# tchen-research/new_cg_variants

Hardware: NVIDIA B200
Metric: CG iterations/s (pr_pcg, Jacobi, 3-D Poisson 256^3) (higher is better)
Workload: dtype f64

## Files before the change

### new_cg_variants_b200/csrc/cgx.cu

```cuda
#include <dlfcn.h>

#include "cgx_launch.cuh"

typedef CUresult (*EncodeTiledFn)(CUtensorMap*, CUtensorMapDataType, cuuint32_t, void*, const cuuint64_t*,
                                  const cuuint64_t*, const cuuint32_t*, const cuuint32_t*,
                                  CUtensorMapInterleave, CUtensorMapSwizzle, CUtensorMapL2promotion,
                                  CUtensorMapFloatOOBfill);
static EncodeTiledFn get_encode_tiled() {
  static EncodeTiledFn fn = nullptr;
  if (!fn) {
    void* p = nullptr;
    cudaDriverEntryPointQueryResult q;
    if (cudaGetDriverEntryPoint("cuTensorMapEncodeTiled", &p, cudaEnableDefault, &q) == cudaSuccess &&
        q == cudaDriverEntryPointSuccess)
      fn = (EncodeTiledFn)p;
  }
  return fn;
}

static thread_local std::string g_err;


int cgx_fail(int code, const char* fmt, ...) {
  char buf[512];
// ... 399 lines not shown

void launch_halo_push(cgx_ctx* c, Args g, const double* v, int ch) { launch_halo_push2(c, g, v, nullptr, ch); }
void launch_halo_push2(cgx_ctx* c, Args g, const double* v0, const double* v1, int ch) {
  if (c->dist.world <= 1) return;
  Plan p;
  p.hout_n = v1 ? 2 : 1; p.hout_ch = ch;
  plan_apply(c, g, p);
  g.halo_ll = 0;
  const double* vs[2] = {v0, v1};
  for (int i = 0; i < p.hout_n; ++i) {
    g.hout_ch = ch + i;
    g.hout_n = 1;
    if (c->dist.csr) {
      const int total = c->dist.send_ptr[c->dist.world];
      if (total > 0) { csr_halo_push_kernel<<<grid_for(c, total), kBlock, 0, c->stream>>>(g, vs[i]); c->launches++; }
    } else {
      halo_push_kernel<<<grid_for(c, c->dist.plane), kBlock, 0, c->stream>>>(g, vs[i]);
      c->launches++;
    }
  }
  plan_commit(c, g, p);
}

bool tma_encode_dims(double* ptr, i64 nx, i64 ny, i64 nz, CUtensorMap* out) {
  EncodeTiledFn enc = get_encode_tiled();
  if (!enc || !ptr) return false;
  cuuint64_t gdim[3] = {(cuuint64_t)nx, (cuuint64_t)ny, (cuuint64_t)nz};
  cuuint64_t gstr[2] = {(cuuint64_t)nx * 8, (cuuint64_t)nx * ny * 8};
  cuuint32_t box[3] = {(cuuint32_t)kPX, (cuuint32_t)kPY, 1};
  cuuint32_t estr[3] = {1, 1, 1};
  return enc(out, CU_TENSOR_MAP_DATA_TYPE_FLOAT64, 3, ptr, gdim, gstr, box, estr,
             CU_TENSOR_MAP_INTERLEAVE_NONE, CU_TENSOR_MAP_SWIZZLE_NONE,
             CU_TENSOR_MAP_L2_PROMOTION_L2_256B, CU_TENSOR_MAP_FLOAT_OOB_FILL_NONE) == CUDA_SUCCESS;
}

static bool tma_prepare_geom(cgx_ctx* c) {
  if (c->op_kind != 2 || c->no_tma) return false;
  const StencilOp& S = c->sten;
  if (S.nx % 2 != 0 || S.nx < 2) return false;
  if (S.ny < 4 && S.nz > 1) return false;
  if (!get_encode_tiled()) return false;
  TmaGeom& G = c->geom;
  G.nx = S.nx; G.ny = S.ny; G.nz = S.nz;
  G.ntx = (S.nx + kTX - 1) / kTX; G.nty = (S.ny + kTY - 1) / kTY;
  G.has_zlo = S.has_zlo; G.has_zhi = S.has_zhi;
  G.diag = S.diag; G.off = S.off;
  G.err = c->d_tma_err;
  G.nchunk = 1;
  G.march_y = 0;
  if (S.nz == 1 && !S.has_zlo && !S.has_zhi && G.nty > 1) {
    G.march_y = 1;
    G.nz = G.nty;
// ... 392 lines not shown
                c->tmap_ok[variant == CGX_CG ? V_R : V_W] &&
                c->pm != 1 && !c->no_elide && !(variant == CGX_GV && (gv_sched || c->gv_manual));
  c->launches_run = 0; c->loop_ms = 0.0;
  c->pend.clear();
  c->pr_fused = false; c->fpar = 0;
  for (int ch = 0; ch < 3; ++ch) c->hepoch[ch] = std::max(c->hepoch[ch], c->fepoch);
  if ((variant == CGX_PR || variant == CGX_M) && path == CGX_PATH_STREAM && !c->no_fused) {
    int frc = cgx_fused_prepare(c);
    if (frc) return frc;
  }
  return CGX_OK;
}

static int begin_finish(cgx_ctx* c, i64 launches0) {
  CU(cudaSetDevice(c->device));
  CU(cudaStreamSynchronize(c->stream));
  CU(cudaGetLastError());
  float ms0 = 0.f;
  CU(cudaEventElapsedTime(&ms0, c->ev[0], c->ev[1]));
  c->setup_ms = ms0;
  if (c->profile) { c->prof_cls.clear(); c->prof_used = 0; }
  c->launches_run = c->launches - launches0;
  c->ran = true;
  return CGX_OK;
}

static int check_device_flags(cgx_ctx* c, const char* who) {
  if (c->use_tma || c->op_kind == 1) {
    int flag = 0;
    CU(cudaMemcpy(&flag, c->d_tma_err, sizeof(int), cudaMemcpyDeviceToHost));
    if (flag) return fail(CGX_ERR_CUDA, "%s: an in-kernel pipeline wait (TMA plane copy / CSR product slot) did not complete within 1 s", who);
  }
  if (c->dist.world > 1 && c->d_win) {
    int err = 0;
    CU(cudaMemcpy(&err, c->d_win + offsetof(WinHdr, error), sizeof(int), cudaMemcpyDeviceToHost));
    if (err) return fail(CGX_ERR_CUDA, "%s: rank %d waited more than 10 s for a peer (halo or scalar exchange)",
                         who, c->dist.rank);
  }
  return CGX_OK;
}

static int group_begin(cgx_ctx** cs, int count, int variant, int max_iter, unsigned hist_mask, int path) {
  for (int i = 0; i < count; ++i)
    if (cs[i] && cs[i]->dist.world > 1 && cs[i]->tol > 0.0)
      return fail(CGX_ERR_UNSUPPORTED, "cgx_begin: a tolerance stops single-GPU solves only (rank %d of a partition has one set)",
                  cs[i]->dist.rank);
// ... 344 lines not shown
  Scal h;
  CU(cudaMemcpy(&h, c->d_sc + c->scpar, sizeof(Scal), cudaMemcpyDeviceToHost));
  info->setup_ms = c->setup_ms; info->loop_ms = c->loop_ms;
  info->h2d_bytes = 0; info->d2h_bytes = 0;
  info->kernel_launches = c->launches_run;
  info->iterations = c->cur_k;
  info->breakdown_iter = h.breakdown;
  info->path = c->path;
  info->stop_iter = c->stop_k;
  return CGX_OK;
}

extern "C" int cgx_set_option(cgx_ctx* c, const char* name, int value) {
  if (!c || !name) return fail(CGX_ERR_ARG, "cgx_set_option: bad arguments");
  if (!strcmp(name, "tma")) { c->no_tma = (value == 0); return CGX_OK; }
  if (!strcmp(name, "csr_stream")) { c->no_csr_stream = (value == 0); return CGX_OK; }
  if (!strcmp(name, "csr_bulk")) { c->csr_bulk = value; return CGX_OK; }
  if (!strcmp(name, "csr_bulk_ring")) { c->csr_bulk_ring = std::max(0, std::min(value, (int)kCbMaxRing)); return CGX_OK; }
  if (!strcmp(name, "csr_bulk_sum")) { c->csr_bulk_sum = value; return CGX_OK; }
  if (!strcmp(name, "csr_bulk_ctas")) { c->csr_bulk_ctas = std::max(1, std::min(value, 4)); return CGX_OK; }
  if (!strcmp(name, "csr_slab")) { c->no_slab = (value == 0); return CGX_OK; }
  if (!strcmp(name, "cg_elide")) { c->no_elide = (value == 0); return CGX_OK; }
  if (!strcmp(name, "pr_fused")) { c->no_fused = (value == 0); return CGX_OK; }
  if (!strcmp(name, "gv_manual")) { c->gv_manual = value != 0; return CGX_OK; }
  if (!strcmp(name, "fused_min_planes")) { c->fused_min_planes = std::max(1, value); return CGX_OK; }
  if (!strcmp(name, "pdl")) { c->pdl_mode = value; return CGX_OK; }
  if (!strcmp(name, "l2_keep")) { c->l2_keep = value; return CGX_OK; }
  if (!strcmp(name, "fused_min_slab")) { c->fused_min_slab = std::max(1, value); return CGX_OK; }
  if (!strcmp(name, "fused_chunks")) { c->fused_chunks = std::max(0, value); return CGX_OK; }
  if (!strcmp(name, "persistent_threshold")) { c->pers_threshold = value; return CGX_OK; }
  if (!strcmp(name, "pers_threads")) { c->pers_threads = value; return CGX_OK; }
  if (!strcmp(name, "pers_ctas")) { c->pers_ctas = value; return CGX_OK; }
  if (!strcmp(name, "debug_skip")) { c->dbg = value; return CGX_OK; }
  if (!strcmp(name, "tma_min_planes")) { c->tma_min_planes = value; return CGX_OK; }
  if (!strcmp(name, "ew_one_wave")) { c->one_wave = value != 0; return CGX_OK; }
  if (!strcmp(name, "stub_allreduce")) {
    if (c->dist.world <= 1) return fail(CGX_ERR_ARG, "cgx_set_option: stub_allreduce needs a partitioned run");
    if (value) { if (c->dist.mode != 3) { c->dist.saved_mode = c->dist.mode; c->dist.mode = 3; } }
    else if (c->dist.mode == 3) c->dist.mode = c->dist.saved_mode;
    return CGX_OK;
  }
  return fail(CGX_ERR_ARG, "cgx_set_option: unknown option '%s'", name);
}

extern "C" int cgx_set_tolerance(cgx_ctx* c, double rtol) {
  if (!c) return fail(CGX_ERR_ARG, "cgx_set_tolerance: ctx is NULL");
// ... 106 lines not shown
  if (info) *info = tmp;
  return tmp.breakdown_iter >= 0 ? CGX_ERR_BREAKDOWN : CGX_OK;
}

static int fetch(cgx_ctx* c, double* x, double* hist, cudaMemcpyKind kind) {
  if (!c || !c->ran) return fail(CGX_ERR_ARG, "cgx_fetch: nothing has been run");
  CU(cudaSetDevice(c->device));
  if (x) CU(cudaMemcpyAsync(x, c->vec[V_X], sizeof(double) * c->n, kind, c->stream));
  if (hist) CU(cudaMemcpyAsync(hist, c->d_hist, sizeof(double) * CGX_HIST_ROWS * (size_t)c->hist_len, kind, c->stream));
  CU(cudaStreamSynchronize(c->stream));
  return CGX_OK;
}
extern "C" int cgx_fetch_host(cgx_ctx* c, double* x, double* hist) { return fetch(c, x, hist, cudaMemcpyDeviceToHost); }
extern "C" int cgx_fetch_dev(cgx_ctx* c, double* x, double* hist) { return fetch(c, x, hist, cudaMemcpyDeviceToDevice); }

extern "C" int cgx_fetch_vector_host(cgx_ctx* c, const char* name, double* out) {
  if (!c || !c->ran || !name || !out) return fail(CGX_ERR_ARG, "cgx_fetch_vector_host: bad arguments");
  for (int i = 0; i < V_COUNT; ++i)
    if (!strcmp(name, kVecNames[i])) {
      if (!c->vec[i]) return fail(CGX_ERR_ARG, "cgx_fetch_vector_host: vector '%s' is not part of the last variant's state", name);
      CU(cudaSetDevice(c->device));
      if (((i == V_RT && c->variant == CGX_CG) || (i == V_WT && c->variant == CGX_GV)) && c->cg_elide && c->cur_k > 0) {
        launch_scale(c, c->d_dinv, c->vec[i == V_RT ? V_R : V_W], c->vec[i]);
        CU(cudaStreamSynchronize(c->stream));
      }
      CU(cudaMemcpy(out, cgx_cur_vec(c, i), sizeof(double) * c->n, cudaMemcpyDeviceToHost));
      return CGX_OK;
    }
  return fail(CGX_ERR_ARG, "cgx_fetch_vector_host: unknown vector '%s'", name);
}

extern "C" int cgx_solve_host(cgx_ctx* c, int variant, const double* b, const double* x0,
                              const double* xt, int64_t n, int max_iter, unsigned hist_mask,
                              int path, double* x, double* hist, cgx_info* info) {
  int rc = load_problem(c, b, x0, xt, n, cudaMemcpyHostToDevice);
  if (rc) return rc;
  int rrc = cgx_run(c, variant, max_iter, hist_mask, path, info);
  if (rrc != CGX_OK && rrc != CGX_ERR_BREAKDOWN) return rrc;
  rc = cgx_fetch_host(c, x, hist);
  if (rc) return rc;
  if (info) {
    info->h2d_bytes = (double)sizeof(double) * n * (xt ? 3 : 2);
    info->d2h_bytes = (double)sizeof(double) * ((x ? n : 0) + (hist ? (i64)CGX_HIST_ROWS * max_iter : 0));
  }
  return rrc;
}
// ... 169 lines not shown
```

### new_cg_variants_b200/csrc/cgx_fused.cu

```cuda
#include "cgx_host.h"
#include "cgx_stencil_fused.cuh"

static const int kFusedVec[3] = {V_P, V_S, V_RT};

double* cgx_cur_vec(cgx_ctx* c, int v) {
  if (c->pr_fused && (c->fpar & 1))
    for (int j = 0; j < 3; ++j)
      if (kFusedVec[j] == v) return c->alt[j];
  return c->vec[v];
}

int cgx_fused_prepare(cgx_ctx* c) {
  c->pr_fused = false;
  c->fpar = 0;
  if (c->op_kind != 2 || !c->use_tma || c->pm == 1) return CGX_OK;
  if (c->dist.world > 1 && (c->dist.mode == 2 || !c->halo_ll)) return CGX_OK;
  if (c->dist.world > 1 && c->sten.nz < c->fused_min_slab) return CGX_OK;
  const StencilOp& S = c->sten;
  for (int j = 0; j < 3; ++j) {
    if (!c->alt[j]) CU(cudaMalloc(&c->alt[j], sizeof(double) * c->n));
    if (!tma_encode_dims(c->vec[kFusedVec[j]], S.nx, S.ny, S.nz, &c->ftmap[0][j])) return CGX_OK;
    if (!tma_encode_dims(c->alt[j], S.nx, S.ny, S.nz, &c->ftmap[1][j])) return CGX_OK;
  }
  for (int ch = 0; ch < 3; ++ch) c->fepoch = std::max(c->fepoch, c->hepoch[ch]);
  if (c->dist.world > 1 && !c->d_gscr) CU(cudaMalloc(&c->d_gscr, sizeof(double) * 4 * (size_t)c->dist.plane));
  c->pr_fused = true;
  return CGX_OK;
}

template <int PM, bool MEUR, bool DIST>
static void launch_fused_t(cgx_ctx* c, const Args& g, int cur) {
  const size_t smem = fused_smem_bytes();
  const int per_sm = ctx_occupancy(c, (const void*)pr_fused_kernel<PM, MEUR, DIST>, kFThreads, smem);
  TmaGeom G = c->geom;
  const int cap = per_sm * c->sm_count, ncols = G.ntx * G.nty;
  G.nchunk = std::max(1, std::min(cap / std::max(1, ncols), G.nz / std::max(1, c->fused_min_planes)));
  if (c->fused_chunks > 0) G.nchunk = std::min(c->fused_chunks, G.nz);
  const int grid = (int)std::min<i64>((i64)ncols * G.nchunk, cap);
  launch_k(pr_fused_kernel<PM, MEUR, DIST>, grid, kFThreads, smem, c->stream, use_pdl(c), c->ftmap[cur][0], c->ftmap[cur][1],
           c->ftmap[cur][2], G, g);
}

void cgx_launch_pr_fused(cgx_ctx* c, Args g) {
  const int cur = c->fpar, nxt = cur ^ 1;
  g.p = nxt ? c->alt[0] : c->vec[V_P];
  g.s = nxt ? c->alt[1] : c->vec[V_S];
  g.rt = nxt ? c->alt[2] : c->vec[V_RT];
  const bool dist = c->dist.world > 1;
  g.gscr = c->d_gscr;
  Plan p;
  p.consume = true;
  p.produce = FK_PIPE;
  plan_apply(c, g, p);
  if (dist) {
    g.hin_epoch = c->fepoch; g.hin_par = (int)(g.hin_epoch & 1);
    g.hout_epoch = c->fepoch + 1; g.hout_par = (int)(g.hout_epoch & 1);
  }
  {
    ProfScope ps(c, PC_FUSED);
    const bool meur = c->variant == CGX_M;
#define CGX_FUSED_GO(PM, D) do { if (meur) launch_fused_t<PM, true, D>(c, g, cur); else launch_fused_t<PM, false, D>(c, g, cur); } while (0)
    if (c->pm == 2) { if (dist) CGX_FUSED_GO(2, true); else CGX_FUSED_GO(2, false); }
    else { if (dist) CGX_FUSED_GO(0, true); else CGX_FUSED_GO(0, false); }
// ... 18 lines not shown
```

### new_cg_variants_b200/csrc/cgx_host.h

```cpp
#pragma once
#include <cuda_runtime.h>

#include <algorithm>
#include <cmath>
#include <cstdarg>
#include <cstdio>
#include <cstring>
#include <functional>
#include <map>
#include <string>
#include <type_traits>
#include <utility>
#include <vector>

#include "../../include/cgx.h"
#include "cgx_kernels.cuh"
#include "cgx_stencil_tma.cuh"
#include "cgx_csr_bulk.cuh"
#include "cgx_persistent.cuh"

using namespace cgx;

int cgx_fail(int code, const char* fmt, ...);
#define fail cgx_fail
// ... 89 lines not shown
  bool peer_ipc[kMaxWorld] = {};
  bool dist_ready = false;
  cudaStream_t own_stream = nullptr;
  u64 epoch = 0;
  u64 hepoch[kChan] = {};
  u64 fepoch = 0;
  int scpar = 0;
  struct Pend { u64 e; int kind; int k; };
  std::vector<Pend> pend;
  void* nccl_comm = nullptr;
  cudaStream_t comm_stream = nullptr;
  cudaEvent_t ev_prod[kSlots] = {}, ev_red[kSlots] = {};
  double* d_nccl = nullptr;
  double* d_ppart = nullptr;
  u64* d_pbar = nullptr;
  PersOut* d_pout = nullptr;
  void* d_prank = nullptr;
  void* d_pbatch = nullptr;
  size_t pbatch_bytes = 0;
  double* d_exp[2][2] = {};
  int pers_threshold = 1 << 19;
  int pers_threads = 0, pers_ctas = 0;
  bool pr_fused = false, no_fused = false;
  int fpar = 0;
  double* alt[3] = {};
  double* d_gscr = nullptr;
  CUtensorMap ftmap[2][3];
  int pdl_mode = 1;
  int l2_keep = -1;
  int fused_min_slab = 64;
  int fused_min_planes = 8, fused_chunks = 0;
  unsigned capture = 0, capture_req = 0;
  double* d_cap[3] = {};
  std::vector<uint8_t> gv_replace;
  bool gv_manual = false;
  int cur_stage = 0;
  std::map<std::pair<const void*, size_t>, int> occ;
  int* d_tma_err = nullptr;
  int variant = 0, max_iter = 0, cur_k = 0, path = CGX_PATH_STREAM;
  double tol = 0.0, run_tol = 0.0;
  int stop_k = -1;
  int* h_stop = nullptr;
  cudaEvent_t ev_stop[2] = {nullptr, nullptr};
  i64 launches_run = 0;
  double setup_ms = 0.0, loop_ms = 0.0;
};
// ... 38 lines not shown
VecIn vec_in(cgx_ctx* c, const double* v, int ch, const Args& g);

int ctx_occupancy(cgx_ctx* c, const void* fn, int threads, size_t smem);

template <class... KArgs, class... Args>
inline cudaError_t launch_k(void (*kern)(KArgs...), int grid, int block, size_t smem, cudaStream_t st, bool pdl, Args&&... args) {
  cudaLaunchConfig_t cfg = {};
  cfg.gridDim = dim3(grid); cfg.blockDim = dim3(block); cfg.dynamicSmemBytes = smem; cfg.stream = st;
  cudaLaunchAttribute at[1];
  at[0].id = cudaLaunchAttributeProgrammaticStreamSerialization;
  at[0].val.programmaticStreamSerializationAllowed = 1;
  cfg.attrs = at; cfg.numAttrs = pdl ? 1 : 0;
  return cudaLaunchKernelEx(&cfg, kern, std::forward<Args>(args)...);
}

inline bool use_pdl(const cgx_ctx* c) { return c->pdl_mode == 2 || (c->pdl_mode == 1 && c->dist.world <= 1); }

inline size_t tma_smem_bytes(int nv) { return stencil_smem_bytes(nv); }

constexpr int kTolChunk = 32;

inline bool csr_dist(const cgx_ctx* c) { return c->dist.world > 1 && c->dist.csr; }
inline int core_stages(const cgx_ctx* c) { return c->pr_fused ? 1 : (c->variant == CGX_HS ? 3 : 2) + (csr_dist(c) ? 1 : 0); }
bool tma_encode_dims(double* ptr, i64 nx, i64 ny, i64 nz, CUtensorMap* out);
int cgx_fused_prepare(cgx_ctx* c);
void cgx_launch_pr_fused(cgx_ctx* c, Args g);
void cgx_fused_push_initial_halo(cgx_ctx* c);
double* cgx_cur_vec(cgx_ctx* c, int v);

void launch_halo_push(cgx_ctx* c, Args g, const double* v, int ch);
void launch_halo_push2(cgx_ctx* c, Args g, const double* v0, const double* v1, int ch);
void launch_instrument(cgx_ctx* c, Args g);
void launch_hist_consume(cgx_ctx* c, Args g);
void launch_capture(cgx_ctx* c, const Args& g);

struct VariantInfo {
  bool meurant, pipe, recompute;
  int cls;
  unsigned need;
};
VariantInfo variant_info(int v, bool prec);

void cgx_iter_stage_pm0(cgx_ctx* c, int s, const Args& g);
void cgx_iter_stage_pm1(cgx_ctx* c, int s, const Args& g);
void cgx_iter_stage_pm2(cgx_ctx* c, int s, const Args& g);

struct PersGeom { int T, nb, R, nslot, slab_cap; unsigned vmask; size_t smem; bool ok; };
// ... 8 lines not shown
```

### new_cg_variants_b200/csrc/cgx_stencil_fused.cuh

```cuda
#pragma once
#include "cgx_stencil_tma.cuh"

namespace cgx {

constexpr int kFStages = 2;
constexpr int kFRing = 4;
constexpr int kFConsumers = 256;
constexpr int kFThreads = kFConsumers + 32;
constexpr int kFPairs = kTX / 64;

__host__ __device__ constexpr size_t fused_smem_bytes() {
  return (size_t)(kFStages * 3 + kFRing) * kPlaneStride * sizeof(double) + 128;
}

__device__ __forceinline__ void named_bar_sync(int id, int nthreads) {
  asm volatile("bar.sync %0, %1;" ::"r"(id), "r"(nthreads) : "memory");
}
__device__ __forceinline__ double2 lds2(const double* p) { return *reinterpret_cast<const double2*>(p); }
__device__ __forceinline__ void sts2(double* p, double a, double b) { *reinterpret_cast<double2*>(p) = make_double2(a, b); }

template <int PM, bool MEUR, bool DIST>
__global__ void __launch_bounds__(kFThreads, 2)
pr_fused_kernel(const __grid_constant__ CUtensorMap tm_p, const __grid_constant__ CUtensorMap tm_s,
                const __grid_constant__ CUtensorMap tm_rt, const TmaGeom G, const Args g) {
  extern __shared__ __align__(128) unsigned char smem_raw[];
  double* smem = reinterpret_cast<double*>(smem_raw + ((128u - (smem_u32(smem_raw) & 127u)) & 127u));
  double* stage = smem;
  double* ring = smem + (size_t)kFStages * 3 * kPlaneStride;
  __shared__ __align__(8) uint64_t full_bar[kFStages], empty_bar[kFStages];

  const int tid = threadIdx.x;
  if (g.tol_on) {
    pdl_launch_dependents();
    pdl_wait();
    if (after_stop(g)) return;
  }
  if (tid == 0) {
#pragma unroll
    for (int s = 0; s < kFStages; ++s) { mbar_init(&full_bar[s], 1); mbar_init(&empty_bar[s], kFConsumers / 32); }
    asm volatile("fence.mbarrier_init.release.cluster;" ::: "memory");
  }
  __syncthreads();
  pdl_launch_dependents();
  pdl_wait();

  double a, b;
  if constexpr (DIST) {
    __shared__ double sh_ab[2];
    if (tid < kFConsumers) {
      if (tid < 32) dist_fold(g, MEUR, sh_ab);
      named_bar_sync(1, kFConsumers);
      a = sh_ab[0]; b = sh_ab[1];
    } else { a = b = 0.0; }
  } else { a = g.sc->a; b = g.sc->b; }
  const double ds = g.dinv_s;
  auto M = [&](double v) { return PM == 2 ? mul_(ds, v) : v; };

  const int zmin = G.has_zlo ? -1 : 0, zmax = G.has_zhi ? G.nz : G.nz - 1;
  const int ncols = G.ntx * G.nty;
  const int nunits = ncols * G.nchunk;
  constexpr uint32_t kBytes = (uint32_t)(3 * kPlane * 8);

  double red[kNRed] = {0.0, 0.0, 0.0, 0.0};

  if (tid >= kFConsumers) {
    if (tid == kFConsumers) {
      uint32_t li = 0;
      for (int unit = blockIdx.x; unit < nunits; unit += gridDim.x) {
        const int col = unit % ncols, chunk = unit / ncols;
        const int z0 = (int)((i64)chunk * G.nz / G.nchunk), z1 = (int)((i64)(chunk + 1) * G.nz / G.nchunk);
        const int x0 = (col % G.ntx) * kTX, y0 = (col / G.ntx) * kTY;
        const int lo = G.march_y ? z0 : max(z0 - 1, zmin), hi = G.march_y ? z1 - 1 : min(z1, zmax);
        for (int zz = lo; zz <= hi; ++zz) {
          if (zz < 0 || zz >= G.nz) continue;
          const int slot = li % kFStages;
          if (li >= kFStages) mbar_wait(&empty_bar[slot], ((li / kFStages) - 1) & 1u, G.err);
          double* dst = stage + (size_t)slot * 3 * kPlaneStride;
          mbar_arrive_expect_tx(&full_bar[slot], kBytes);
          const int ty0 = G.march_y ? zz * kTY : y0, tz = G.march_y ? 0 : zz;
          tma_load_3d(dst, &tm_p, x0 - 2, ty0 - 1, tz, &full_bar[slot]);
          tma_load_3d(dst + kPlaneStride, &tm_s, x0 - 2, ty0 - 1, tz, &full_bar[slot]);
          tma_load_3d(dst + 2 * kPlaneStride, &tm_rt, x0 - 2, ty0 - 1, tz, &full_bar[slot]);
          ++li;
        }
      }
    }
  } else {
    const int ly = tid >> 5, lx = tid & 31;
    uint32_t li = 0;
    bool first_seg = true;
    for (int unit = blockIdx.x; unit < nunits; unit += gridDim.x) {
      const int col = unit % ncols, chunk = unit / ncols;
      const int z0 = (int)((i64)chunk * G.nz / G.nchunk), z1 = (int)((i64)(chunk + 1) * G.nz / G.nchunk);
      const int x0 = (col % G.ntx) * kTX, y0 = (col / G.ntx) * kTY;
      const int lo = G.march_y ? z0 : max(z0 - 1, zmin), hi = G.march_y ? z1 - 1 : min(z1, zmax);
      if (!first_seg) named_bar_sync(1, kFConsumers);
      first_seg = false;

      typedef double Set[kFPairs][2];
      const int step_stride = G.march_y ? kTY * G.nx : G.nx * G.ny;
      const int idx0 = (G.march_y ? ly : y0 + ly) * G.nx + x0 + 2 * lx;
      const int ybase = G.march_y ? ly : y0 + ly, ystep = G.march_y ? kTY : 0;
      bool okx[kFPairs];
#pragma unroll
      for (int j = 0; j < kFPairs; ++j) okx[j] = (x0 + 2 * lx + 64 * j) < G.nx;
      const int rlo = DIST ? max(lo, 0) : lo, rhi = DIST ? min(hi, G.nz - 1) : hi;
      auto fetch_xr = [&](int z, Set& xs, Set& rs) {
        const bool oky = ybase + z * ystep < G.ny;
        const int ib = idx0 + z * step_stride;
#pragma unroll
        for (int j = 0; j < kFPairs; ++j) {
          const int i = (oky && okx[j]) ? ib + 64 * j : 0;
          const double2 xv = *reinterpret_cast<const double2*>(g.x + i);
          const double2 rv = *reinterpret_cast<const double2*>(g.r + i);
          xs[j][0] = xv.x; xs[j][1] = xv.y; rs[j][0] = rv.x; rs[j][1] = rv.y;
        }
      };

      auto plane_step = [&](const int zz, Set& xc, Set& rc, Set& xn, Set& rn, Set& rnew, Set& rold) {
        if (zz <= rhi) {
          const bool fullp = zz >= z0 && zz < z1;
          if (zz + 1 >= z0 && zz + 1 < z1) fetch_xr(zz + 1, xn, rn);
          const int slot = li % kFStages;
          mbar_wait(&full_bar[slot], (li / kFStages) & 1u, G.err);
          const double* sp = stage + (size_t)slot * 3 * kPlaneStride;
          const double* ss = sp + kPlaneStride;
          const double* srt = sp + 2 * kPlaneStride;
          double* pn = ring + (size_t)(zz & (kFRing - 1)) * kPlaneStride;
          const bool oky = ybase + zz * ystep < G.ny;
          const int ib = idx0 + zz * step_stride;
#pragma unroll
          for (int j = 0; j < kFPairs; ++j) {
            const int c = (ly + 1) * kPX + 2 * lx + 64 * j + 2;
            const double2 po = lds2(sp + c), so = lds2(ss + c), rto = lds2(srt + c);
            const double pov[2] = {po.x, po.y}, sov[2] = {so.x, so.y}, rtov[2] = {rto.x, rto.y};
            double xo[2], rtn[2], pnw[2];
            const bool ok = fullp && oky && okx[j];
#pragma unroll
            for (int l = 0; l < 2; ++l) {
              rtn[l] = axmy_(rtov[l], a, M(sov[l]));
              pnw[l] = axpy_(rtn[l], b, pov[l]);
            }
            sts2(pn + c, pnw[0], pnw[1]);
            if (ok) {
#pragma unroll
              for (int l = 0; l < 2; ++l) {
                xo[l] = axpy_(xc[j][l], a, pov[l]);
                rnew[j][l] = axmy_(rc[j][l], a, sov[l]);
                red[3] = fma(rtn[l], rnew[j][l], red[3]);
              }
              const int i = ib + 64 * j;
              *reinterpret_cast<double2*>(g.x + i) = make_double2(xo[0], xo[1]);
              *reinterpret_cast<double2*>(g.r + i) = make_double2(rnew[j][0], rnew[j][1]);
              *reinterpret_cast<double2*>(g.rt + i) = make_double2(rtn[0], rtn[1]);
              *reinterpret_cast<double2*>(g.p + i) = make_double2(pnw[0], pnw[1]);
            }
          }
          if (fullp) {
            if (tid < 2 * (kTX / 2)) {
              const int py = (tid >= kTX / 2) ? kPY - 1 : 0;
              const int c = py * kPX + 2 * (tid & (kTX / 2 - 1)) + 2;
              const double2 po = lds2(sp + c), so = lds2(ss + c), rto = lds2(srt + c);
              const double r0 = axmy_(rto.x, a, M(so.x)), r1 = axmy_(rto.y, a, M(so.y));
              sts2(pn + c, axpy_(r0, b, po.x), axpy_(r1, b, po.y));
            } else if (tid < kTX + 2 * kTY) {
              const int u = tid - kTX;
              const int c = ((u % kTY) + 1) * kPX + ((u >= kTY) ? kTX + 2 : 1);
              const double r0 = axmy_(srt[c], a, M(ss[c]));
              pn[c] = axpy_(r0, b, sp[c]);
            }
          }
          __syncwarp();
          if (lx == 0) mbar_arrive(&empty_bar[slot]);
          ++li;
        } else if constexpr (DIST) {
          if (hi >= G.nz) {
            double* pn = ring + (size_t)(G.nz & (kFRing - 1)) * kPlaneStride + (ly + 1) * kPX + 2 * lx + 2;
#pragma unroll
            for (int j = 0; j < kFPairs; ++j) {
              const int e = (ybase < G.ny && okx[j]) ? idx0 + 64 * j : 0;
              const double2 t = *reinterpret_cast<const double2*>(g.gscr + e);
              sts2(pn + 64 * j, t.x, t.y);
            }
          }
        }
        named_bar_sync(1, kFConsumers);

        const int q = zz - 1;
        if (q >= z0 && q < z1) {
          const double* pm = ring + (size_t)((q - 1) & (kFRing - 1)) * kPlaneStride;
          const double* pc = ring + (size_t)(q & (kFRing - 1)) * kPlaneStride;
          const double* pp = ring + (size_t)((q + 1) & (kFRing - 1)) * kPlaneStride;
          const bool has_zm = !G.march_y && ((q > 0) || G.has_zlo);
          const bool has_zp = !G.march_y && ((q < G.nz - 1) || G.has_zhi);
          const bool oky = ybase + q * ystep < G.ny;
          const int ib = idx0 + q * step_stride;
#pragma unroll
          for (int j = 0; j < kFPairs; ++j) {
            if (oky && okx[j]) {
              const int c = (ly + 1) * kPX + 2 * lx + 64 * j + 2;
              const double2 zm = lds2(pm + c), zp = lds2(pp + c);
              const double2 ym = lds2(pc + c - kPX), yp = lds2(pc + c + kPX), ct = lds2(pc + c);
              const double xm = pc[c - 1], xp = pc[c + 2];
              const double zmv[2] = {zm.x, zm.y}, zpv[2] = {zp.x, zp.y}, ymv[2] = {ym.x, ym.y}, ypv[2] = {yp.x, yp.y},
                           ctv[2] = {ct.x, ct.y}, xmv[2] = {xm, ct.x}, xpv[2] = {ct.y, xp};
              double y[2];
#pragma unroll
              for (int l = 0; l < 2; ++l) {
                double acc = 0.0, t;
                t = add_(acc, mul_(G.off, zmv[l]));          acc = has_zm ? t : acc;
                acc = add_(acc, mul_(G.off, ymv[l]));
                acc = add_(acc, mul_(G.off, xmv[l]));
                acc = add_(acc, mul_(G.diag, ctv[l]));
                acc = add_(acc, mul_(G.off, xpv[l]));
                acc = add_(acc, mul_(G.off, ypv[l]));
                t = add_(acc, mul_(G.off, zpv[l]));          acc = has_zp ? t : acc;
                y[l] = acc;
                const double sti = M(acc);
                red[0] = fma(ctv[l], acc, red[0]);
                red[1] = fma(rold[j][l], sti, red[1]);
                red[2] = fma(sti, acc, red[2]);
              }
              *reinterpret_cast<double2*>(g.s + ib + 64 * j) = make_double2(y[0], y[1]);
            }
          }
        }
      };

      Set xa, ra, xb, rb, rna = {}, rnb = {};
      if (rlo >= z0) fetch_xr(rlo, xa, ra);
      if constexpr (DIST) {
        int* err = &g.d.win[g.d.rank]->error;
        const size_t chs = ghl_off(g.d, 1, 0, 0);
#pragma unroll 1
        for (int side = 0; side < 2; ++side) {
          if (side == 0 ? lo >= 0 : hi < G.nz) continue;
          const u64* gh = g.d.ghl + ghl_off(g.d, 0, g.hin_par, side);
#pragma unroll 1
          for (int j = 0; j < kFPairs; ++j) {
            if (!(ybase < G.ny && okx[j])) continue;
            const int e = idx0 + 64 * j;
            double pnw[2] = {0.0, 0.0};
            if (!(g.dbg & 1)) {
              LLReq rq[3][2];
#pragma unroll
              for (int v = 0; v < 3; ++v)
#pragma unroll
                for (int l = 0; l < 2; ++l) { rq[v][l].src = gh + v * chs + 2 * (size_t)(e + l); ll_issue(rq[v][l]); }
#pragma unroll
              for (int l = 0; l < 2; ++l) {
                const double po = ll_finish(rq[0][l], g.hin_epoch, err), so = ll_finish(rq[1][l], g.hin_epoch, err),
                             rto = ll_finish(rq[2][l], g.hin_epoch, err);
                pnw[l] = axpy_(axmy_(rto, a, M(so)), b, po);
              }
            }
            if (side == 0) sts2(ring + (size_t)((-1) & (kFRing - 1)) * kPlaneStride + (ly + 1) * kPX + 2 * lx + 64 * j + 2, pnw[0], pnw[1]);
            else *reinterpret_cast<double2*>(g.gscr + e) = make_double2(pnw[0], pnw[1]);
          }
        }
      }
      for (int zz = rlo; zz <= rhi + 1; zz += 2) {
        plane_step(zz, xa, ra, xb, rb, rna, rnb);
        if (zz + 1 <= rhi + 1) plane_step(zz + 1, xb, rb, xa, ra, rnb, rna);
      }
      if constexpr (DIST) {
        if (!(g.dbg & 1)) {
          const size_t chs = ghl_off(g.d, 1, 0, 0);
          const double* src[3] = {g.p, g.s, g.rt};
#pragma unroll 1
          for (int side = 0; side < 2; ++side) {
            if (side == 0 ? !(z0 == 0 && g.d.has_lo) : !(z1 == G.nz && g.d.has_hi)) continue;
            u64* dst = (side == 0 ? g.d.ghl_lo : g.d.ghl_hi) + ghl_off(g.d, 0, g.hout_par, side ^ 1);
            const int i0 = idx0 + (side == 0 ? 0 : (G.nz - 1) * step_stride);
#pragma unroll 1
            for (int j = 0; j < kFPairs; ++j) {
              if (!(ybase < G.ny && okx[j])) continue;
#pragma unroll
              for (int v = 0; v < 3; ++v) {
                const double2 t = *reinterpret_cast<const double2*>(src[v] + i0 + 64 * j);
                ll_store(dst + v * chs + 2 * (size_t)(idx0 + 64 * j), t.x, g.hout_epoch);
                ll_store(dst + v * chs + 2 * (size_t)(idx0 + 64 * j + 1), t.y, g.hout_epoch);
              }
            }
          }
        }
      }
    }
// ... 23 lines not shown
```

Measured before the change: 4386.

## Recompute s = A·p in fused PR kernel instead of storing and reloading it

After: 3897, median of 6. -11.1%, worse.

```diff
diff --git a/new_cg_variants_b200/csrc/cgx.cu b/new_cg_variants_b200/csrc/cgx.cu
--- a/new_cg_variants_b200/csrc/cgx.cu
+++ b/new_cg_variants_b200/csrc/cgx.cu
@@ -445,12 +445,12 @@
   plan_commit(c, g, p);
 }
 
-bool tma_encode_dims(double* ptr, i64 nx, i64 ny, i64 nz, CUtensorMap* out) {
+bool tma_encode_dims(double* ptr, i64 nx, i64 ny, i64 nz, CUtensorMap* out, int box_y) {
   EncodeTiledFn enc = get_encode_tiled();
   if (!enc || !ptr) return false;
   cuuint64_t gdim[3] = {(cuuint64_t)nx, (cuuint64_t)ny, (cuuint64_t)nz};
   cuuint64_t gstr[2] = {(cuuint64_t)nx * 8, (cuuint64_t)nx * ny * 8};
-  cuuint32_t box[3] = {(cuuint32_t)kPX, (cuuint32_t)kPY, 1};
+  cuuint32_t box[3] = {(cuuint32_t)kPX, (cuuint32_t)(box_y > 0 ? box_y : kPY), 1};
   cuuint32_t estr[3] = {1, 1, 1};
   return enc(out, CU_TENSOR_MAP_DATA_TYPE_FLOAT64, 3, ptr, gdim, gstr, box, estr,
              CU_TENSOR_MAP_INTERLEAVE_NONE, CU_TENSOR_MAP_SWIZZLE_NONE,
@@ -889,6 +889,10 @@
   if (c->profile) { c->prof_cls.clear(); c->prof_used = 0; }
   c->launches_run = c->launches - launches0;
   c->ran = true;
+  if (c->poison_s && c->pr_fused && c->dist.world <= 1) {
+    CU(cudaMemset(c->vec[V_S], 0xff, sizeof(double) * c->n));
+    CU(cudaMemset(c->alt[1], 0xff, sizeof(double) * c->n));
+  }
   return CGX_OK;
 }
 
@@ -1279,6 +1283,7 @@
   if (!strcmp(name, "csr_slab")) { c->no_slab = (value == 0); return CGX_OK; }
   if (!strcmp(name, "cg_elide")) { c->no_elide = (value == 0); return CGX_OK; }
   if (!strcmp(name, "pr_fused")) { c->no_fused = (value == 0); return CGX_OK; }
+  if (!strcmp(name, "fused_poison_s")) { c->poison_s = value != 0; return CGX_OK; }
   if (!strcmp(name, "gv_manual")) { c->gv_manual = value != 0; return CGX_OK; }
   if (!strcmp(name, "fused_min_planes")) { c->fused_min_planes = std::max(1, value); return CGX_OK; }
   if (!strcmp(name, "pdl")) { c->pdl_mode = value; return CGX_OK; }
@@ -1431,6 +1436,15 @@
       CU(cudaSetDevice(c->device));
       if (((i == V_RT && c->variant == CGX_CG) || (i == V_WT && c->variant == CGX_GV)) && c->cg_elide && c->cur_k > 0) {
         launch_scale(c, c->d_dinv, c->vec[i == V_RT ? V_R : V_W], c->vec[i]);
+        CU(cudaStreamSynchronize(c->stream));
+      }
+      if (i == V_S && c->pr_fused && c->cur_k > 0) {
+        if (c->dist.world > 1)
+          return fail(CGX_ERR_UNSUPPORTED, "cgx_fetch_vector_host: s of a rank of a partition after a single-launch "
+                      "PR / M run is not stored (rebuilding it needs the neighbours' planes of p)");
+        Args g = make_args(c);
+        g.tol_on = 0;
+        launch_spmv<SP_PLAIN, 0, false>(c, g, cgx_cur_vec(c, V_P), cgx_cur_vec(c, V_S));
         CU(cudaStreamSynchronize(c->stream));
       }
       CU(cudaMemcpy(out, cgx_cur_vec(c, i), sizeof(double) * c->n, cudaMemcpyDeviceToHost));
diff --git a/new_cg_variants_b200/csrc/cgx_fused.cu b/new_cg_variants_b200/csrc/cgx_fused.cu
--- a/new_cg_variants_b200/csrc/cgx_fused.cu
+++ b/new_cg_variants_b200/csrc/cgx_fused.cu
@@ -19,8 +19,10 @@
   const StencilOp& S = c->sten;
   for (int j = 0; j < 3; ++j) {
     if (!c->alt[j]) CU(cudaMalloc(&c->alt[j], sizeof(double) * c->n));
-    if (!tma_encode_dims(c->vec[kFusedVec[j]], S.nx, S.ny, S.nz, &c->ftmap[0][j])) return CGX_OK;
-    if (!tma_encode_dims(c->alt[j], S.nx, S.ny, S.nz, &c->ftmap[1][j])) return CGX_OK;
+    if (kFusedVec[j] == V_S) continue;
+    const int box_y = kFusedVec[j] == V_P ? kFPY : kPY;
+    if (!tma_encode_dims(c->vec[kFusedVec[j]], S.nx, S.ny, S.nz, &c->ftmap[0][j], box_y)) return CGX_OK;
+    if (!tma_encode_dims(c->alt[j], S.nx, S.ny, S.nz, &c->ftmap[1][j], box_y)) return CGX_OK;
   }
   for (int ch = 0; ch < 3; ++ch) c->fepoch = std::max(c->fepoch, c->hepoch[ch]);
   if (c->dist.world > 1 && !c->d_gscr) CU(cudaMalloc(&c->d_gscr, sizeof(double) * 4 * (size_t)c->dist.plane));
@@ -37,8 +39,8 @@
   G.nchunk = std::max(1, std::min(cap / std::max(1, ncols), G.nz / std::max(1, c->fused_min_planes)));
   if (c->fused_chunks > 0) G.nchunk = std::min(c->fused_chunks, G.nz);
   const int grid = (int)std::min<i64>((i64)ncols * G.nchunk, cap);
-  launch_k(pr_fused_kernel<PM, MEUR, DIST>, grid, kFThreads, smem, c->stream, use_pdl(c), c->ftmap[cur][0], c->ftmap[cur][1],
-           c->ftmap[cur][2], G, g);
+  launch_k(pr_fused_kernel<PM, MEUR, DIST>, grid, kFThreads, smem, c->stream, use_pdl(c), c->ftmap[cur][0], c->ftmap[cur][2],
+           G, g);
 }
 
 void cgx_launch_pr_fused(cgx_ctx* c, Args g) {
diff --git a/new_cg_variants_b200/csrc/cgx_host.h b/new_cg_variants_b200/csrc/cgx_host.h
--- a/new_cg_variants_b200/csrc/cgx_host.h
+++ b/new_cg_variants_b200/csrc/cgx_host.h
@@ -135,6 +135,7 @@
   int pers_threshold = 1 << 19;
   int pers_threads = 0, pers_ctas = 0;
   bool pr_fused = false, no_fused = false;
+  bool poison_s = false;
   int fpar = 0;
   double* alt[3] = {};
   double* d_gscr = nullptr;
@@ -219,7 +220,7 @@
 
 inline bool csr_dist(const cgx_ctx* c) { return c->dist.world > 1 && c->dist.csr; }
 inline int core_stages(const cgx_ctx* c) { return c->pr_fused ? 1 : (c->variant == CGX_HS ? 3 : 2) + (csr_dist(c) ? 1 : 0); }
-bool tma_encode_dims(double* ptr, i64 nx, i64 ny, i64 nz, CUtensorMap* out);
+bool tma_encode_dims(double* ptr, i64 nx, i64 ny, i64 nz, CUtensorMap* out, int box_y = 0);
 int cgx_fused_prepare(cgx_ctx* c);
 void cgx_launch_pr_fused(cgx_ctx* c, Args g);
 void cgx_fused_push_initial_halo(cgx_ctx* c);
diff --git a/new_cg_variants_b200/csrc/cgx_stencil_fused.cuh b/new_cg_variants_b200/csrc/cgx_stencil_fused.cuh
--- a/new_cg_variants_b200/csrc/cgx_stencil_fused.cuh
+++ b/new_cg_variants_b200/csrc/cgx_stencil_fused.cuh
@@ -3,14 +3,18 @@
 
 namespace cgx {
 
-constexpr int kFStages = 2;
+constexpr int kFPRing = 4;
+constexpr int kFRtStages = 2;
 constexpr int kFRing = 4;
+constexpr int kFPY = kTY + 4;
+constexpr int kFPPlane = kPX * kFPY;
+constexpr int kFPStride = ((kFPPlane * 8 + 127) / 128) * 128 / 8;
 constexpr int kFConsumers = 256;
 constexpr int kFThreads = kFConsumers + 32;
 constexpr int kFPairs = kTX / 64;
 
 __host__ __device__ constexpr size_t fused_smem_bytes() {
-  return (size_t)(kFStages * 3 + kFRing) * kPlaneStride * sizeof(double) + 128;
+  return ((size_t)kFPRing * kFPStride + (size_t)(kFRtStages + kFRing) * kPlaneStride) * sizeof(double) + 128;
 }
 
 __device__ __forceinline__ void named_bar_sync(int id, int nthreads) {
@@ -19,15 +23,93 @@
 __device__ __forceinline__ double2 lds2(const double* p) { return *reinterpret_cast<const double2*>(p); }
 __device__ __forceinline__ void sts2(double* p, double a, double b) { *reinterpret_cast<double2*>(p) = make_double2(a, b); }
 
+__device__ __forceinline__ void row_sum2(const double* pm, const double* pc, const double* pp, int q, bool has_zm,
+                                         bool has_zp, double diag, double off, double (&y)[2], double (&ctv)[2]) {
+  const double2 zm = lds2(pm + q), zp = lds2(pp + q);
+  const double2 ym = lds2(pc + q - kPX), yp = lds2(pc + q + kPX), ct = lds2(pc + q);
+  const double xm = pc[q - 1], xp = pc[q + 2];
+  const double zmv[2] = {zm.x, zm.y}, zpv[2] = {zp.x, zp.y}, ymv[2] = {ym.x, ym.y}, ypv[2] = {yp.x, yp.y},
+               xmv[2] = {xm, ct.x}, xpv[2] = {ct.y, xp};
+  ctv[0] = ct.x; ctv[1] = ct.y;
+#pragma unroll
+  for (int l = 0; l < 2; ++l) {
+    double acc = 0.0, t;
+    t = add_(acc, mul_(off, zmv[l]));          acc = has_zm ? t : acc;
+    acc = add_(acc, mul_(off, ymv[l]));
+    acc = add_(acc, mul_(off, xmv[l]));
+    acc = add_(acc, mul_(diag, ctv[l]));
+    acc = add_(acc, mul_(off, xpv[l]));
+    acc = add_(acc, mul_(off, ypv[l]));
+    t = add_(acc, mul_(off, zpv[l]));          acc = has_zp ? t : acc;
+    y[l] = acc;
+  }
+}
+__device__ __forceinline__ double row_sum1(const double* pm, const double* pc, const double* pp, int q, bool has_zm,
+                                           bool has_zp, double diag, double off) {
+  double acc = 0.0, t;
+  t = add_(acc, mul_(off, pm[q]));             acc = has_zm ? t : acc;
+  acc = add_(acc, mul_(off, pc[q - kPX]));
+  acc = add_(acc, mul_(off, pc[q - 1]));
+  acc = add_(acc, mul_(diag, pc[q]));
+  acc = add_(acc, mul_(off, pc[q + 1]));
+  acc = add_(acc, mul_(off, pc[q + kPX]));
+  t = add_(acc, mul_(off, pp[q]));             acc = has_zp ? t : acc;
+  return acc;
+}
+
+static __device__ __noinline__ void fused_fill_ghost(double* dst, const u64* gh, int* err, u64 epoch, bool off, int x0, int y0,
+                                              int nx, int ny) {
+  const int tid = threadIdx.x, ly = tid >> 5, lx = tid & 31;
+  constexpr int kN = 2 * kFPairs + 2;
+  int cq[kN], xq[kN], yq[kN];
+  bool mine[kN];
+#pragma unroll
+  for (int j = 0; j < kFPairs; ++j)
+#pragma unroll
+    for (int l2 = 0; l2 < 2; ++l2) {
+      cq[2 * j + l2] = (ly + 1) * kPX + 2 * lx + 64 * j + 2 + l2;
+      xq[2 * j + l2] = x0 + 2 * lx + 64 * j + l2; yq[2 * j + l2] = y0 + ly;
+      mine[2 * j + l2] = true;
+    }
+  if (tid < kTX) {
+    const int py = (tid >= kTX / 2) ? kPY - 1 : 0, xx = 2 * (tid & (kTX / 2 - 1));
+#pragma unroll
+    for (int l2 = 0; l2 < 2; ++l2) {
+      cq[kN - 2 + l2] = py * kPX + xx + 2 + l2; xq[kN - 2 + l2] = x0 + xx + l2; yq[kN - 2 + l2] = y0 - 1 + py;
+      mine[kN - 2 + l2] = true;
+    }
+  } else {
+    const int uu = tid - kTX;
+    cq[kN - 2] = ((uu % kTY) + 1) * kPX + ((uu >= kTY) ? kTX + 2 : 1);
+    xq[kN - 2] = (uu >= kTY) ? x0 + kTX : x0 - 1; yq[kN - 2] = y0 + uu % kTY;
+    mine[kN - 2] = tid < kTX + 2 * kTY;
+    cq[kN - 1] = 0; xq[kN - 1] = -1; yq[kN - 1] = -1; mine[kN - 1] = false;
+  }
+  LLReq rq[kN];
+  bool in[kN];
+#pragma unroll
+  for (int k = 0; k < kN; ++k) {
+    in[k] = mine[k] && !off && xq[k] >= 0 && xq[k] < nx && yq[k] >= 0 && yq[k] < ny;
+    rq[k].src = gh + 2 * (size_t)(in[k] ? yq[k] * nx + xq[k] : 0);
+    if (in[k]) ll_issue(rq[k]);
+  }
+#pragma unroll
+  for (int k = 0; k < kN; ++k) {
+    const double v = in[k] ? ll_finish(rq[k], epoch, err) : 0.0;
+    if (mine[k]) dst[cq[k]] = v;
+  }
+}
+
 template <int PM, bool MEUR, bool DIST>
 __global__ void __launch_bounds__(kFThreads, 2)
-pr_fused_kernel(const __grid_constant__ CUtensorMap tm_p, const __grid_constant__ CUtensorMap tm_s,
-                const __grid_constant__ CUtensorMap tm_rt, const TmaGeom G, const Args g) {
+pr_fused_kernel(const __grid_constant__ CUtensorMap tm_p, const __grid_constant__ CUtensorMap tm_rt, const TmaGeom G,
+                const Args g) {
   extern __shared__ __align__(128) unsigned char smem_raw[];
   double* smem = reinterpret_cast<double*>(smem_raw + ((128u - (smem_u32(smem_raw) & 127u)) & 127u));
-  double* stage = smem;
-  double* ring = smem + (size_t)kFStages * 3 * kPlaneStride;
-  __shared__ __align__(8) uint64_t full_bar[kFStages], empty_bar[kFStages];
+  double* pring = smem;
+  double* rtst = pring + (size_t)kFPRing * kFPStride;
+  double* ring = rtst + (size_t)kFRtStages * kPlaneStride;
+  __shared__ __align__(8) uint64_t pfull[kFPRing], pempty[kFPRing], rfull[kFRtStages], rempty[kFRtStages];
 
   const int tid = threadIdx.x;
   if (g.tol_on) {
@@ -37,7 +119,9 @@
   }
   if (tid == 0) {
 #pragma unroll
-    for (int s = 0; s < kFStages; ++s) { mbar_init(&full_bar[s], 1); mbar_init(&empty_bar[s], kFConsumers / 32); }
+    for (int s = 0; s < kFPRing; ++s) { mbar_init(&pfull[s], 1); mbar_init(&pempty[s], kFConsumers / 32); }
+#pragma unroll
+    for (int s = 0; s < kFRtStages; ++s) { mbar_init(&rfull[s], 1); mbar_init(&rempty[s], kFConsumers / 32); }
     asm volatile("fence.mbarrier_init.release.cluster;" ::: "memory");
   }
   __syncthreads();
@@ -59,41 +143,55 @@
   const int zmin = G.has_zlo ? -1 : 0, zmax = G.has_zhi ? G.nz : G.nz - 1;
   const int ncols = G.ntx * G.nty;
   const int nunits = ncols * G.nchunk;
-  constexpr uint32_t kBytes = (uint32_t)(3 * kPlane * 8);
+  constexpr uint32_t kPBytes = (uint32_t)(kFPPlane * 8), kRtBytes = (uint32_t)(kPlane * 8);
+  struct Span { int z0, z1, x0, y0, lo, hi, rlo, rhi, plo, phi; };
+  auto span = [&](int unit) {
+    Span u;
+    const int col = unit % ncols, chunk = unit / ncols;
+    u.z0 = (int)((i64)chunk * G.nz / G.nchunk); u.z1 = (int)((i64)(chunk + 1) * G.nz / G.nchunk);
+    u.x0 = (col % G.ntx) * kTX; u.y0 = (col / G.ntx) * kTY;
+    u.lo = G.march_y ? u.z0 : max(u.z0 - 1, zmin); u.hi = G.march_y ? u.z1 - 1 : min(u.z1, zmax);
+    u.rlo = max(u.lo, 0); u.rhi = min(u.hi, G.nz - 1);
+    u.plo = G.march_y ? u.rlo : max(u.rlo - 1, zmin); u.phi = G.march_y ? u.rhi : min(u.rhi + 1, zmax);
+    return u;
+  };
 
   double red[kNRed] = {0.0, 0.0, 0.0, 0.0};
 
   if (tid >= kFConsumers) {
     if (tid == kFConsumers) {
-      uint32_t li = 0;
+      uint32_t lp = 0, lr = 0;
       for (int unit = blockIdx.x; unit < nunits; unit += gridDim.x) {
-        const int col = unit % ncols, chunk = unit / ncols;
-        const int z0 = (int)((i64)chunk * G.nz / G.nchunk), z1 = (int)((i64)(chunk + 1) * G.nz / G.nchunk);
-        const int x0 = (col % G.ntx) * kTX, y0 = (col / G.ntx) * kTY;
-        const int lo = G.march_y ? z0 : max(z0 - 1, zmin), hi = G.march_y ? z1 - 1 : min(z1, zmax);
-        for (int zz = lo; zz <= hi; ++zz) {
-          if (zz < 0 || zz >= G.nz) continue;
-          const int slot = li % kFStages;
-          if (li >= kFStages) mbar_wait(&empty_bar[slot], ((li / kFStages) - 1) & 1u, G.err);
-          double* dst = stage + (size_t)slot * 3 * kPlaneStride;
-          mbar_arrive_expect_tx(&full_bar[slot], kBytes);
-          const int ty0 = G.march_y ? zz * kTY : y0, tz = G.march_y ? 0 : zz;
-          tma_load_3d(dst, &tm_p, x0 - 2, ty0 - 1, tz, &full_bar[slot]);
-          tma_load_3d(dst + kPlaneStride, &tm_s, x0 - 2, ty0 - 1, tz, &full_bar[slot]);
-          tma_load_3d(dst + 2 * kPlaneStride, &tm_rt, x0 - 2, ty0 - 1, tz, &full_bar[slot]);
-          ++li;
+        const Span u = span(unit);
+        auto ty0_of = [&](int zz) { return G.march_y ? zz * kTY : u.y0; };
+        int pnext = u.plo;
+        for (int zz = u.rlo; zz <= u.rhi; ++zz) {
+          for (; pnext <= min(G.march_y ? zz : zz + 1, u.phi); ++pnext, ++lp) {
+            const int slot = lp % kFPRing;
+            if (lp >= kFPRing) mbar_wait(&pempty[slot], ((lp / kFPRing) - 1) & 1u, G.err);
+            if (pnext < 0 || pnext >= G.nz) {
+              mbar_arrive(&pfull[slot]);
+            } else {
+              mbar_arrive_expect_tx(&pfull[slot], kPBytes);
+              tma_load_3d(pring + (size_t)slot * kFPStride, &tm_p, u.x0 - 2, ty0_of(pnext) - 2, G.march_y ? 0 : pnext,
+                          &pfull[slot]);
+            }
+          }
+          const int slot = lr % kFRtStages;
+          if (lr >= kFRtStages) mbar_wait(&rempty[slot], ((lr / kFRtStages) - 1) & 1u, G.err);
+          mbar_arrive_expect_tx(&rfull[slot], kRtBytes);
+          tma_load_3d(rtst + (size_t)slot * kPlaneStride, &tm_rt, u.x0 - 2, ty0_of(zz) - 1, G.march_y ? 0 : zz, &rfull[slot]);
+          ++lr;
         }
       }
     }
   } else {
     const int ly = tid >> 5, lx = tid & 31;
-    uint32_t li = 0;
+    uint32_t lp = 0, lr = 0;
     bool first_seg = true;
     for (int unit = blockIdx.x; unit < nunits; unit += gridDim.x) {
-      const int col = unit % ncols, chunk = unit / ncols;
-      const int z0 = (int)((i64)chunk * G.nz / G.nchunk), z1 = (int)((i64)(chunk + 1) * G.nz / G.nchunk);
-      const int x0 = (col % G.ntx) * kTX, y0 = (col / G.ntx) * kTY;
-      const int lo = G.march_y ? z0 : max(z0 - 1, zmin), hi = G.march_y ? z1 - 1 : min(z1, zmax);
+      const Span u = span(unit);
+      const int z0 = u.z0, z1 = u.z1, x0 = u.x0, y0 = u.y0, lo = u.lo, hi = u.hi;
       if (!first_seg) named_bar_sync(1, kFConsumers);
       first_seg = false;
 
@@ -104,7 +202,7 @@
       bool okx[kFPairs];
 #pragma unroll
       for (int j = 0; j < kFPairs; ++j) okx[j] = (x0 + 2 * lx + 64 * j) < G.nx;
-      const int rlo = DIST ? max(lo, 0) : lo, rhi = DIST ? min(hi, G.nz - 1) : hi;
+      const int rlo = u.rlo, rhi = u.rhi;
       auto fetch_xr = [&](int z, Set& xs, Set& rs) {
         const bool oky = ybase + z * ystep < G.ny;
         const int ib = idx0 + z * step_stride;
@@ -117,25 +215,54 @@
         }
       };
 
+      const uint32_t Pbase = lp;
+      int pw = 0, prl = 0;
+      auto pslot = [&](int z) { return pring + (size_t)((Pbase + (uint32_t)(z - u.plo)) % kFPRing) * kFPStride; };
+      auto wait_p = [&](int upto) {
+        while (u.plo + pw <= upto) {
+          const uint32_t l = Pbase + (uint32_t)pw;
+          mbar_wait(&pfull[l % kFPRing], (l / kFPRing) & 1u, G.err);
+          if constexpr (DIST) {
+            const int z = u.plo + pw;
+            if (z < 0 || z >= G.nz)
+              fused_fill_ghost(pring + (size_t)(l % kFPRing) * kFPStride + kPX, g.d.ghl + ghl_off(g.d, 0, g.hin_par, z < 0 ? 0 : 1),
+                               &g.d.win[g.d.rank]->error, g.hin_epoch, (g.dbg & 1) != 0, x0, y0, G.nx, G.ny);
+          }
+          ++pw;
+        }
+      };
+      auto release_p = [&](int upto) {
+        __syncwarp();
+        for (; u.plo + prl <= upto; ++prl)
+          if (lx == 0) mbar_arrive(&pempty[(Pbase + (uint32_t)prl) % kFPRing]);
+      };
+
       auto plane_step = [&](const int zz, Set& xc, Set& rc, Set& xn, Set& rn, Set& rnew, Set& rold) {
         if (zz <= rhi) {
           const bool fullp = zz >= z0 && zz < z1;
           if (zz + 1 >= z0 && zz + 1 < z1) fetch_xr(zz + 1, xn, rn);
-          const int slot = li % kFStages;
-          mbar_wait(&full_bar[slot], (li / kFStages) & 1u, G.err);
-          const double* sp = stage + (size_t)slot * 3 * kPlaneStride;
-          const double* ss = sp + kPlaneStride;
-          const double* srt = sp + 2 * kPlaneStride;
+          wait_p(min(G.march_y ? zz : zz + 1, u.phi));
+          const int slot = lr % kFRtStages;
+          mbar_wait(&rfull[slot], (lr / kFRtStages) & 1u, G.err);
+          const double* srt = rtst + (size_t)slot * kPlaneStride;
+          const double* om = pslot(zz - 1) + kPX;
+          const double* oc = pslot(zz) + kPX;
+          const double* op = pslot(zz + 1) + kPX;
+          const bool has_zm = !G.march_y && ((zz > 0) || G.has_zlo);
+          const bool has_zp = !G.march_y && ((zz < G.nz - 1) || G.has_zhi);
           double* pn = ring + (size_t)(zz & (kFRing - 1)) * kPlaneStride;
           const bool oky = ybase + zz * ystep < G.ny;
           const int ib = idx0 + zz * step_stride;
 #pragma unroll
           for (int j = 0; j < kFPairs; ++j) {
             const int c = (ly + 1) * kPX + 2 * lx + 64 * j + 2;
-            const double2 po = lds2(sp + c), so = lds2(ss + c), rto = lds2(srt + c);
-            const double pov[2] = {po.x, po.y}, sov[2] = {so.x, so.y}, rtov[2] = {rto.x, rto.y};
+            const bool in = oky && okx[j];
+            double so[2], pov[2];
+            row_sum2(om, oc, op, c, has_zm, has_zp, G.diag, G.off, so, pov);
+            const double2 rto = lds2(srt + c);
+            const double sov[2] = {in ? so[0] : 0.0, in ? so[1] : 0.0}, rtov[2] = {rto.x, rto.y};
             double xo[2], rtn[2], pnw[2];
-            const bool ok = fullp && oky && okx[j];
+            const bool ok = fullp && in;
 #pragma unroll
             for (int l = 0; l < 2; ++l) {
               rtn[l] = axmy_(rtov[l], a, M(sov[l]));
@@ -157,22 +284,30 @@
             }
           }
           if (fullp) {
+            const int ty0 = G.march_y ? zz * kTY : y0;
             if (tid < 2 * (kTX / 2)) {
-              const int py = (tid >= kTX / 2) ? kPY - 1 : 0;
-              const int c = py * kPX + 2 * (tid & (kTX / 2 - 1)) + 2;
-              const double2 po = lds2(sp + c), so = lds2(ss + c), rto = lds2(srt + c);
-              const double r0 = axmy_(rto.x, a, M(so.x)), r1 = axmy_(rto.y, a, M(so.y));
-              sts2(pn + c, axpy_(r0, b, po.x), axpy_(r1, b, po.y));
+              const int py = (tid >= kTX / 2) ? kPY - 1 : 0, xx = 2 * (tid & (kTX / 2 - 1));
+              const int c = py * kPX + xx + 2;
+              const bool in = x0 + xx < G.nx && ty0 - 1 + py >= 0 && ty0 - 1 + py < G.ny;
+              double so[2], po[2];
+              row_sum2(om, oc, op, c, has_zm, has_zp, G.diag, G.off, so, po);
+              const double2 rto = lds2(srt + c);
+              const double r0 = axmy_(rto.x, a, M(in ? so[0] : 0.0)), r1 = axmy_(rto.y, a, M(in ? so[1] : 0.0));
+              sts2(pn + c, axpy_(r0, b, po[0]), axpy_(r1, b, po[1]));
             } else if (tid < kTX + 2 * kTY) {
-              const int u = tid - kTX;
-              const int c = ((u % kTY) + 1) * kPX + ((u >= kTY) ? kTX + 2 : 1);
-              const double r0 = axmy_(srt[c], a, M(ss[c]));
-              pn[c] = axpy_(r0, b, sp[c]);
+              const int uu = tid - kTX;
+              const int c = ((uu % kTY) + 1) * kPX + ((uu >= kTY) ? kTX + 2 : 1);
+              const int xh = (uu >= kTY) ? x0 + kTX : x0 - 1;
+              const bool in = xh >= 0 && xh < G.nx && ty0 + uu % kTY < G.ny;
+              const double so = row_sum1(om, oc, op, c, has_zm, has_zp, G.diag, G.off);
+              const double r0 = axmy_(srt[c], a, M(in ? so : 0.0));
+              pn[c] = axpy_(r0, b, oc[c]);
             }
           }
           __syncwarp();
-          if (lx == 0) mbar_arrive(&empty_bar[slot]);
-          ++li;
+          if (lx == 0) mbar_arrive(&rempty[slot]);
+          ++lr;
+          release_p(G.march_y ? zz : zz - 1);
         } else if constexpr (DIST) {
           if (hi >= G.nz) {
             double* pn = ring + (size_t)(G.nz & (kFRing - 1)) * kPlaneStride + (ly + 1) * kPX + 2 * lx + 2;
@@ -195,33 +330,22 @@
           const bool has_zp = !G.march_y && ((q < G.nz - 1) || G.has_zhi);
           const bool oky = ybase + q * ystep < G.ny;
           const int ib = idx0 + q * step_stride;
+          bool keep_s = false;
+          if constexpr (DIST) keep_s = (q == 0 && g.d.has_lo) || (q == G.nz - 1 && g.d.has_hi);
 #pragma unroll
           for (int j = 0; j < kFPairs; ++j) {
             if (oky && okx[j]) {
               const int c = (ly + 1) * kPX + 2 * lx + 64 * j + 2;
-              const double2 zm = lds2(pm + c), zp = lds2(pp + c);
-              const double2 ym = lds2(pc + c - kPX), yp = lds2(pc + c + kPX), ct = lds2(pc + c);
-              const double xm = pc[c - 1], xp = pc[c + 2];
-              const double zmv[2] = {zm.x, zm.y}, zpv[2] = {zp.x, zp.y}, ymv[2] = {ym.x, ym.y}, ypv[2] = {yp.x, yp.y},
-                           ctv[2] = {ct.x, ct.y}, xmv[2] = {xm, ct.x}, xpv[2] = {ct.y, xp};
-              double y[2];
+              double y[2], ctv[2];
+              row_sum2(pm, pc, pp, c, has_zm, has_zp, G.diag, G.off, y, ctv);
 #pragma unroll
               for (int l = 0; l < 2; ++l) {
-                double acc = 0.0, t;
-                t = add_(acc, mul_(G.off, zmv[l]));          acc = has_zm ? t : acc;
-                acc = add_(acc, mul_(G.off, ymv[l]));
-                acc = add_(acc, mul_(G.off, xmv[l]));
-                acc = add_(acc, mul_(G.diag, ctv[l]));
-                acc = add_(acc, mul_(G.off, xpv[l]));
-                acc = add_(acc, mul_(G.off, ypv[l]));
-                t = add_(acc, mul_(G.off, zpv[l]));          acc = has_zp ? t : acc;
-                y[l] = acc;
-                const double sti = M(acc);
-                red[0] = fma(ctv[l], acc, red[0]);
+                const double sti = M(y[l]);
+                red[0] = fma(ctv[l], y[l], red[0]);
                 red[1] = fma(rold[j][l], sti, red[1]);
-                red[2] = fma(sti, acc, red[2]);
+                red[2] = fma(sti, y[l], red[2]);
               }
-              *reinterpret_cast<double2*>(g.s + ib + 64 * j) = make_double2(y[0], y[1]);
+              if (keep_s) *reinterpret_cast<double2*>(g.s + ib + 64 * j) = make_double2(y[0], y[1]);
             }
           }
         }
@@ -263,6 +387,8 @@
         plane_step(zz, xa, ra, xb, rb, rna, rnb);
         if (zz + 1 <= rhi + 1) plane_step(zz + 1, xb, rb, xa, ra, rnb, rna);
       }
+      release_p(u.phi);
+      lp = Pbase + (uint32_t)(u.phi - u.plo + 1);
       if constexpr (DIST) {
         if (!(g.dbg & 1)) {
           const size_t chs = ghl_off(g.d, 1, 0, 0);
```
